# thomeou/SALSA

Hardware: AMD Instinct MI355X
Metric: SALSA feat-extract audio-s/s (higher is better)
Workload: dtype f64 (STFT, noise-floor tracker, eigen-solve cold list) + packed f32 (covariance and eigen-solve of the certified frames); 1 GPU; Full SALSA FOA (eigenvector path): batch 32x60-s 4-ch 24 kHz clips per GPU, feature-extract only, n_fft 512 hop 300 fmax_doa 9000 cond 5 tracking on; clips_per_gpu=32, feature=salsa, format=foa, clip_groups=default

## Files before the change

include/salsa_hip.h:

```cpp
#ifndef SALSA_HIP_H
#define SALSA_HIP_H

#include <stddef.h>
#include <stdint.h>

#ifdef __cplusplus
extern "C" {
#endif

#define SALSA_ABI_VERSION 2

enum { SALSA_FORMAT_FOA = 0, SALSA_FORMAT_MIC = 1 };
enum { SALSA_FEATURE_SALSA = 0, SALSA_FEATURE_LITE = 1, SALSA_FEATURE_IPD = 2 };
enum { SALSA_LAYOUT_PLANAR = 0, SALSA_LAYOUT_INTERLEAVED = 1 };

enum { SALSA_FLAG_FLEX = 1, SALSA_FLAG_NO_CLIP_FREQS = 2, SALSA_FLAG_CLIP_SPATIAL_ALIAS = 4,
       SALSA_FLAG_FORCE_F64 = 8 };

enum {
    SALSA_OK = 0,
    SALSA_PARTIAL = 1,
    SALSA_EINVAL = -1,
    SALSA_ENFFT = -2,
    SALSA_EFORMAT = -3,
// ... 41 lines not shown

int salsa_logspec_batch(salsa_plan *plan, const float *d_audio, int batch, int n_channels, int64_t n_samples,
                        float *d_out, void *hip_stream);

size_t salsa_eigvec_workspace_bytes(const salsa_plan *plan, int batch, int n_bins, int64_t n_frames);
int salsa_eigvec_batch(salsa_plan *plan, const float *d_X, int batch, int n_bins, int64_t n_frames, int lower_bin,
                       double *d_out, unsigned char *d_gate, void *d_workspace, size_t workspace_bytes,
                       void *hip_stream);

int salsa_eigvec_feature_batch(salsa_plan *plan, const float *d_X, int batch, int n_bins, int64_t n_frames, int lower_bin,
                               float *d_feat, void *d_workspace, size_t workspace_bytes, void *hip_stream);

int salsa_plan_set_fused(salsa_plan *plan, int mode);

int salsa_plan_set_stats(salsa_plan *plan, unsigned long long *d_counters);

int salsa_scaler_accumulate(const float *d_feat, int batch, int n_channels, int64_t n_frames, int n_freq,
                            int n_scaler_channels, double *d_sums, void *hip_stream);
int salsa_normalize_batch(float *d_feat, int batch, int n_channels, int64_t n_frames, int n_freq, int n_scaler_channels,
                          const float *d_mean, const float *d_std, void *hip_stream);

int salsa_plan_set_scaler(salsa_plan *plan, const float *d_mean, const float *d_std);

int salsa_to_freq_major(const float *d_feat, int64_t n_rows, int64_t n_frames, int n_freq, double *d_out, void *hip_stream);

#define SALSA_AUGMENT_NPAR 40
int salsa_augment_batch(const float *d_in, int64_t in_batch_stride, int64_t in_channel_stride, float *d_out, int batch,
                        int64_t n_frames, int n_freq, int audio_format, int n_zero_channels, const int *d_params,
                        const float *d_uval, const float *d_minmax, void *hip_stream);
int salsa_augment_gcc_batch(const float *d_in, int64_t in_batch_stride, int64_t in_channel_stride, float *d_out, int batch,
// ... 104 lines not shown
```

salsa_amd/csrc/build_guard.h:

```cpp
#ifndef SALSA_BUILD_GUARD_H
#define SALSA_BUILD_GUARD_H

#if !defined(SALSA_PROBE_BUILD)
#ifdef BN_PROBE_NO_Y
#error "BN_PROBE_NO_Y is a timing-probe switch: build with -DSALSA_PROBE_BUILD (its results are not the product's)"
#endif
#ifdef CONV_FETCH_COLMAJOR
#error "CONV_FETCH_COLMAJOR is a timing-probe switch: build with -DSALSA_PROBE_BUILD (its results are not the product's)"
#endif
#ifdef CONV_NO_BARRIER
#error "CONV_NO_BARRIER is a timing-probe switch: build with -DSALSA_PROBE_BUILD (its results are not the product's)"
#endif
#ifdef CONV_NO_EPI
#error "CONV_NO_EPI is a timing-probe switch: build with -DSALSA_PROBE_BUILD (its results are not the product's)"
#endif
#ifdef CONV_NO_FETCH
#error "CONV_NO_FETCH is a timing-probe switch: build with -DSALSA_PROBE_BUILD (its results are not the product's)"
#endif
#ifdef CONV_NO_LDSREAD
#error "CONV_NO_LDSREAD is a timing-probe switch: build with -DSALSA_PROBE_BUILD (its results are not the product's)"
#endif
#ifdef CONV_NO_ROW_SHARE
#error "CONV_NO_ROW_SHARE is a timing-probe switch: build with -DSALSA_PROBE_BUILD (its results are not the product's)"
#endif
// ... 21 lines not shown
#ifdef FZ_PROBE_NOSOLVE
#error "FZ_PROBE_NOSOLVE is a timing-probe switch: build with -DSALSA_PROBE_BUILD (its results are not the product's)"
#endif
#ifdef GRU_PROBE_BWD_NO_LOAD
#error "GRU_PROBE_BWD_NO_LOAD is a timing-probe switch: build with -DSALSA_PROBE_BUILD (its results are not the product's)"
#endif
#ifdef GRU_PROBE_BWD_NO_MATVEC
#error "GRU_PROBE_BWD_NO_MATVEC is a timing-probe switch: build with -DSALSA_PROBE_BUILD (its results are not the product's)"
#endif
#ifdef GRU_PROBE_BWD_NO_STORE
#error "GRU_PROBE_BWD_NO_STORE is a timing-probe switch: build with -DSALSA_PROBE_BUILD (its results are not the product's)"
#endif
#ifdef K1_FRAME_MAJOR
#error "K1_FRAME_MAJOR is a timing-probe switch: build with -DSALSA_PROBE_BUILD (its results are not the product's)"
#endif
#ifdef STEM_NO_STORE
#error "STEM_NO_STORE is a timing-probe switch: build with -DSALSA_PROBE_BUILD (its results are not the product's)"
#endif
#ifdef TR_PROBE_NO_CONSUME
#error "TR_PROBE_NO_CONSUME is a timing-probe switch: build with -DSALSA_PROBE_BUILD (its results are not the product's)"
#endif
#ifdef TR_PROBE_NO_PRODUCE
#error "TR_PROBE_NO_PRODUCE is a timing-probe switch: build with -DSALSA_PROBE_BUILD (its results are not the product's)"
#endif
#ifdef WIDE_W_ZERO
#error "WIDE_W_ZERO is a timing-probe switch: build with -DSALSA_PROBE_BUILD (its results are not the product's)"
#endif
#ifdef WIDE_X_ZERO
#error "WIDE_X_ZERO is a timing-probe switch: build with -DSALSA_PROBE_BUILD (its results are not the product's)"
#endif
// ... 203 lines not shown
#endif
#ifdef K1_NF_LITE
#define SALSA_BG_K1_NF_LITE " K1_NF_LITE=" SALSA_BG_STR(K1_NF_LITE)
#else
#define SALSA_BG_K1_NF_LITE ""
#endif
#ifdef K1_SPILL_NT
#define SALSA_BG_K1_SPILL_NT " K1_SPILL_NT=" SALSA_BG_STR(K1_SPILL_NT)
#else
#define SALSA_BG_K1_SPILL_NT ""
#endif
#ifdef K1_STD
#define SALSA_BG_K1_STD " K1_STD=" SALSA_BG_STR(K1_STD)
#else
#define SALSA_BG_K1_STD ""
#endif
#ifdef K3_FT_N
#define SALSA_BG_K3_FT_N " K3_FT_N=" SALSA_BG_STR(K3_FT_N)
#else
#define SALSA_BG_K3_FT_N ""
#endif
#ifdef K3_GATHER_NT
#define SALSA_BG_K3_GATHER_NT " K3_GATHER_NT=" SALSA_BG_STR(K3_GATHER_NT)
#else
#define SALSA_BG_K3_GATHER_NT ""
#endif
#ifdef K3_GROUP
#define SALSA_BG_K3_GROUP " K3_GROUP=" SALSA_BG_STR(K3_GROUP)
#else
#define SALSA_BG_K3_GROUP ""
// ... 213 lines not shown
    SALSA_BG_CONV_SPREAD_FETCH \
    SALSA_BG_CONV_STATS_DOT2 \
    SALSA_BG_CONV_WIDE_STORE \
    SALSA_BG_CONV_WPS \
    SALSA_BG_GRU_FILL \
    SALSA_BG_K1_INTERLEAVE \
    SALSA_BG_K1_LITE_1024_WAVES \
    SALSA_BG_K1_LITE_PAIR_MAJOR \
    SALSA_BG_K1_LITE_STD \
    SALSA_BG_K1_LITE_STD_WAVES \
    SALSA_BG_K1_LITE_WAVES \
    SALSA_BG_K1_NF_FULL \
    SALSA_BG_K1_NF_LITE \
    SALSA_BG_K1_SPILL_NT \
    SALSA_BG_K1_STD \
    SALSA_BG_K3_FT_N \
    SALSA_BG_K3_GATHER_NT \
    SALSA_BG_K3_GROUP \
    SALSA_BG_K3_NT_N \
    SALSA_BG_K3_OUT_NT \
    SALSA_BG_K3_PK_WAVES \
    SALSA_BG_K3_STAGE_LDS \
    SALSA_BG_K3_XCD_CHUNK \
    SALSA_BG_NN_NT_LD \
    SALSA_BG_NN_NT_ST \
    SALSA_BG_SALSA_COL0 \
    SALSA_BG_SALSA_COL0_MIN \
    SALSA_BG_SALSA_GATE_DOUBT \
    SALSA_BG_SALSA_PK \
    SALSA_BG_SALSA_PK_FOA_MIN \
// ... 29 lines not shown
```

salsa_amd/csrc/salsa_internal.h:

```cpp
#pragma once
#include <hip/hip_runtime.h>
#include <stdio.h>

#include "../../include/salsa_hip.h"
#include "salsa_math.h"
#include "salsa_workspace.h"

#define SALSA_LOCAL __attribute__((visibility("hidden")))

extern "C" SALSA_LOCAL void salsa_set_last_error_(const char *msg);

namespace salsa_impl {

static inline int fail(int code, const char *fmt, const char *a = "", long b = 0)
{
    char msg[512];
    snprintf(msg, sizeof(msg), fmt, a, b);
    salsa_set_last_error_(msg);
    return code;
}

static inline int hip_fail(const char *expr, hipError_t e)
{
    char msg[512];
// ... 26 lines not shown
    int format;
    int tracking;
    int n_hop;
    int pair_sel;
    int nch;
    double cond;
    double inv_cond;
    double delta;
    double snr_ratio;
    const float *sc_mean;
    const float *sc_std;
    unsigned long long *stats;
    int force_f64;
    unsigned *doubt32;
    unsigned *doubt_flag;
};

constexpr int FEATURE_LOGSPEC_ONLY = 3;

#ifndef K3_FT_N
#define K3_FT_N 8
#endif
constexpr int K3_FT = K3_FT_N;
#ifndef K3_NT_N
#define K3_NT_N 128
#endif
constexpr int K3_NT = K3_NT_N;
#ifndef SALSA_PK
#define SALSA_PK 1
#endif
#define SALSA_PK_COND_MIN 2.0

__device__ __forceinline__ int swz(int e) { return e ^ ((e >> 3) & 7); }

__device__ __forceinline__ void wave_lds_fence()
{
    __builtin_amdgcn_fence(__ATOMIC_RELEASE, "wavefront");
    __builtin_amdgcn_wave_barrier();
    __builtin_amdgcn_fence(__ATOMIC_ACQUIRE, "wavefront");
}

__device__ __forceinline__ float power32(const float2 x)
{
    const float t = x.x * x.x;
    return __builtin_fmaf(x.y, x.y, t);
}
// ... 11 lines not shown
}

constexpr int SALSA_MAX_GROUPS = 16;

struct salsa_plan {
    salsa_params p;
    int device;
    int lower, upper, cutoff, nd, F, ident;
    int spec_lo, spec_hi, flex;
    double delta, snr_ratio;
    double *d_window;
    double *d_window_doa;
    salsa::cplx<double> *d_tw;
    const float *sc_mean, *sc_std;
    unsigned long long *stats;
    int fused;
    int timing;
    int stop_after;
    int n_kernels;
    hipEvent_t ev0[SALSA_MAX_KERNELS], ev1[SALSA_MAX_KERNELS];
    const char *names[SALSA_MAX_KERNELS];
    int n_groups;
    int pipe_flags;
    hipStream_t streams[SALSA_MAX_GROUPS + 1];
    hipEvent_t ev_fork, ev_stft[SALSA_MAX_GROUPS], ev_stft2[SALSA_MAX_GROUPS], ev_join[SALSA_MAX_GROUPS + 1];
    hipStream_t cap_stream;
    hipGraphExec_t gexec;
    struct GraphKey {
        const float *audio;
        float *out;
        void *ws;
        const float *sc_mean, *sc_std;
        int batch, n_groups, flags;
        int64_t n_samples;
        bool operator==(const GraphKey &o) const
        {
            return audio == o.audio && out == o.out && ws == o.ws && sc_mean == o.sc_mean && sc_std == o.sc_std && batch == o.batch &&
                   n_groups == o.n_groups && flags == o.flags && n_samples == o.n_samples;
        }
    } gkey;
};

namespace salsa_impl {

static inline void bind_workspace(const WorkspaceLayout &L, void *base, int g0, bool with_doubt, float4 *&Xs, unsigned *&valid, KParams &kp)
{
    unsigned char *w = (unsigned char *)base;
    Xs = (float4 *)(w + L.spill_at(g0));
    valid = (unsigned *)(w + L.gate_at(g0));
    kp.doubt32 = with_doubt ? (unsigned *)(w + L.doubt_at(g0)) : nullptr;
    kp.doubt_flag = with_doubt ? (unsigned *)(w + L.flag_at(g0)) : nullptr;
}

// ... 35 lines not shown
```

salsa_amd/csrc/salsa_kernels.hip:

```cpp
#include "build_guard.h"
#include "salsa_internal.h"
#include <type_traits>

using salsa::cplx;
using namespace salsa_impl;

namespace {

template <int N> struct fft_cfg {
    static constexpr int NSUB = (N == 1024) ? 2 : 1;
    static constexpr int NS = N / NSUB;
    static constexpr int R = (NS == 512) ? 8 : 4;
    static constexpr int NP = (NS == 512) ? 2 : 3;
};

template <typename V> __device__ __forceinline__ V ld_off_c(const V *base, unsigned byte_off, int const_bytes) { return *(const V *)((const char *)base + byte_off + const_bytes); }
#ifndef K1_SPILL_NT
#define K1_SPILL_NT 1
#endif
typedef float salsa_f4v __attribute__((ext_vector_type(4)));
#ifndef TR_NT_LD
#define TR_NT_LD 0
#endif
#ifndef K3_GATHER_NT
// ... 644 lines not shown
#endif
constexpr int K3_OW = K3_NT + 8;
#ifndef K3_XCD_CHUNK
#define K3_XCD_CHUNK 16
#endif

#ifndef K3_STAGE_LDS
#define K3_STAGE_LDS 0
#endif
#ifndef K3_OUT_NT
#define K3_OUT_NT 1
#endif
#ifndef K3_PK_WAVES
#define K3_PK_WAVES 4
#endif
template <bool FEAT, int NHOP, bool FAST = false, bool PK = false>
__global__ __launch_bounds__(K3_NT, PK ? K3_PK_WAVES : 1) void cov_eig_kernel(const KParams kp, const float4 *__restrict__ Xs,
                                                      const unsigned *__restrict__ valid32,
                                                      float *__restrict__ out_feat, double *__restrict__ out_eig,
                                                      unsigned char *__restrict__ gate)
{
    constexpr int G = NHOP >= 0 ? K3_GROUP : 1;
    constexpr bool PAIRED = G > 1;
    static_assert(K3_FT % G == 0 && G <= 4 && K3_FT / G <= 16, "work-list entry layout");
    __shared__ unsigned short list[K3_FT * K3_NT];
    __shared__ unsigned short slow[FAST ? K3_FT * K3_NT : 1];
    __shared__ int count, nslow;
    __shared__ __attribute__((aligned(16))) unsigned rowoff[NHOP >= 0 ? K3_FT + 2 * NHOP + 2 : 2];
    __shared__ __attribute__((aligned(16))) float otile[FEAT ? 3 * K3_FT * K3_OW : 4];
#if K3_STAGE_LDS
// ... 98 lines not shown
        const int first = bin0 + K3_OW, tail = kp.F - first;
        for (int i = tid; i < nft * tail; i += K3_NT) {
            const int ft = i / tail, f = first + (i - ft * tail);
#pragma unroll
            for (int c = 0; c < 3; c++) st_off(of, 4u * (unsigned)((c * Tn + t0 + ft) * kp.F + f), 0.f);
        }
    }
    __syncthreads();
    const int n = count;
    const int stride = 2 * kp.nd;
    const int nhop = NHOP >= 0 ? NHOP : kp.n_hop;
    const float4 *xclip = Xs + (long)b * Tn * stride;
    const bool ungated = !kp.tracking && !kp.flex;
    auto solve_emit = [&](const salsa::herm4<double> &R, int t, int bin, auto path) {
        constexpr int PATH = decltype(path)::value;
        const bool foa = kp.format == SALSA_FORMAT_FOA;
        const salsa::eig_result<double> er = salsa::herm4_gate_eigvec<PATH>(R, kp.cond, kp.inv_cond, ungated, !foa);
        if (PATH == 1 && er.fallback) {
            slow[atomicAdd(&nslow, 1)] = (unsigned short)(((t - t0) << 8) | (bin - bin0));
            return;
        }
        if (er.doubt && kp.doubt32 && !ungated) {
            atomicOr(&kp.doubt32[((long)b * ((kp.nd + TR_BINS - 1) / TR_BINS) + (bin >> 5)) * Tn + t], 1u << (bin & 31));
            atomicOr(kp.doubt_flag, 1u);
        }
        double e[3] = {0.0, 0.0, 0.0};
        unsigned char g = er.rank1 ? 2 : 1;
        if (er.rank1 || ungated) {
            const int k = bin + kp.lower;
            const double den = kp.flex ? (double)((float)(k == 0 ? 1 : k) * (float)kp.delta) : kp.delta * (double)k;
            if (PATH != 2 && er.col0) {
                if (foa) salsa::normalise_foa_col0(er.u, e);
                else salsa::normalise_mic_col0(er.u, den, e);
            } else if (PATH != 1) {
                if (foa) salsa::normalise_foa(er.u, e, ungated);
                else salsa::normalise_mic(er.u, den, e);
            }
            g = 2;
        } else if (FEAT && kp.flex && !kp.tracking) {
            e[0] = __builtin_nan("");
        }
        emit(t, bin, e, g);
    };
    using hot_path = std::integral_constant<int, FAST ? 1 : 2>;
    using cold_path = std::integral_constant<int, 2>;
    if constexpr (PK) {
        static_assert(!PK || (G == 2 && FEAT && FAST && NHOP >= 0), "the packed solve takes the two frames of a pair");
        constexpr int NW = 2 * NHOP + 2;
        const unsigned half = 16u * (unsigned)kp.nd;
#if K3_STAGE_LDS
        if (n > 0) {
            for (int i = tid; i < (K3_FT + 6) * 2 * K3_NT; i += K3_NT) {
                const int fr = i / (2 * K3_NT), rem = i - fr * 2 * K3_NT, pr = rem / K3_NT, bl = rem - pr * K3_NT;
                if (bl < nbc) stage[i] = ld_off(xclip, rowoff[fr] + 16u * (unsigned)(bin0 + bl) + (pr ? half : 0u));
            }
// ... 99 lines not shown
        } else {
            salsa::herm4<double> R = {};
            for (int k = -nhop; k <= nhop; k++) {
                int tt = t + k;
                while (tt < 0) tt += Tn;
                while (tt >= Tn) tt -= Tn;
                const float4 a = xb[tt * stride], c = xb[tt * stride + kp.nd];
                const cplx<double> x[4] = {{(double)a.x, (double)a.y}, {(double)a.z, (double)a.w},
                                           {(double)c.x, (double)c.y}, {(double)c.z, (double)c.w}};
                salsa::herm4_rank1_add(R, x);
            }
            solve_emit(R, t, bin, hot_path{});
        }
    }
    if (FAST) {
        __syncthreads();
        const int ns = nslow;
        if (kp.stats && tid == 0) {
            int live = 0;
            for (int s = 0; s < n; s++) live += __popc((list[s] >> 12) & 15);
            atomicAdd(&kp.stats[0], (unsigned long long)n);
            atomicAdd(&kp.stats[1], (unsigned long long)live);
            atomicAdd(&kp.stats[2], (unsigned long long)ns);
            atomicAdd(&kp.stats[3], 1ull);
        }
        for (int s = tid; s < ns; s += K3_NT) {
            const int i = slow[s];
            const int t = t0 + (i >> 8), bin = bin0 + (i & 255);
            const float4 *xb = xclip + bin;
            salsa::herm4<double> R = {};
            for (int k = -nhop; k <= nhop; k++) {
                int tt = t + k;
                while (tt < 0) tt += Tn;
                while (tt >= Tn) tt -= Tn;
                const float4 a = xb[tt * stride], c = xb[tt * stride + kp.nd];
                const cplx<double> x[4] = {{(double)a.x, (double)a.y}, {(double)a.z, (double)a.w},
                                           {(double)c.x, (double)c.y}, {(double)c.z, (double)c.w}};
                salsa::herm4_rank1_add(R, x);
            }
            solve_emit(R, t, bin, cold_path{});
        }
    }
    if (FEAT) {
        __syncthreads();
        const bool vec = !(kp.F & 3) && !(seg & 3) && !(bin0 & 3);
        if (vec) {
            const int q = seg >> 2;
            for (int i = tid; i < 3 * nft * q; i += K3_NT) {
                const int row = i / q, col = i - row * q, c = row / nft, ft = row - c * nft;
                float4 *dst = (float4 *)(of + ((long)(c * Tn + t0 + ft) * kp.F + bin0 + 4 * col));
                const float4 val = *(const float4 *)(otile + (c * K3_FT + ft) * K3_OW + 4 * col);
                if (K3_OUT_NT) st_off_nt(dst, 0u, val);
                else *dst = val;
            }
        } else {
            for (int i = tid; i < 3 * nft * seg; i += K3_NT) {
                const int row = i / seg, col = i - row * seg, c = row / nft, ft = row - c * nft;
                of[(long)(c * Tn + t0 + ft) * kp.F + bin0 + col] = otile[(c * K3_FT + ft) * K3_OW + col];
            }
        }
    }
}

template <bool FEAT>
__global__ __launch_bounds__(256) void gate_doubt_kernel(const KParams kp, const float4 *__restrict__ Xs, float *__restrict__ out_feat,
                                                         double *__restrict__ out_eig, unsigned char *__restrict__ gate)
{
    if (*(const volatile unsigned *)kp.doubt_flag == 0u) return;
    const int Tn = kp.T, n32 = (kp.nd + TR_BINS - 1) / TR_BINS, stride = 2 * kp.nd;
    const long nwords = (long)kp.B * n32 * Tn;
    const bool foa = kp.format == SALSA_FORMAT_FOA;
    for (long wi = (long)blockIdx.x * blockDim.x + threadIdx.x; wi < nwords; wi += (long)gridDim.x * blockDim.x) {
        unsigned word = kp.doubt32[wi];
        if (!word) continue;
        const int t = (int)(wi % Tn), g32 = (int)((wi / Tn) % n32), b = (int)(wi / ((long)Tn * n32));
        while (word) {
            const int j = __ffs((int)word) - 1;
            word &= word - 1u;
            const int bin = 32 * g32 + j;
            const float4 *xb = Xs + (long)b * Tn * stride + bin;
            salsa::herm4<double> R = {};
            for (int k = -kp.n_hop; k <= kp.n_hop; k++) {
                int tt = t + k;
                while (tt < 0) tt += Tn;
                while (tt >= Tn) tt -= Tn;
                const float4 a = xb[tt * stride], c = xb[tt * stride + kp.nd];
                const cplx<double> x[4] = {{(double)a.x, (double)a.y}, {(double)a.z, (double)a.w},
                                           {(double)c.x, (double)c.y}, {(double)c.z, (double)c.w}};
                salsa::herm4_rank1_add(R, x);
            }
            const bool rank1 = salsa::herm4_rank1_by_jacobi(R, kp.cond);
            double e[3] = {0.0, 0.0, 0.0};
            if (rank1) {
                const salsa::eig_result<double> er = salsa::herm4_gate_eigvec<2>(R, kp.cond, kp.inv_cond, true, !foa);
                const int k = bin + kp.lower;
                const double den = kp.flex ? (double)((float)(k == 0 ? 1 : k) * (float)kp.delta) : kp.delta * (double)k;
                if (foa) salsa::normalise_foa(er.u, e, false);
                else salsa::normalise_mic(er.u, den, e);
            } else if (FEAT && kp.flex && !kp.tracking) {
                e[0] = __builtin_nan("");
            }
            if (FEAT) {
#pragma unroll
                for (int i = 0; i < 3; i++) out_feat[(((long)b * kp.OC + 4 + i) * Tn + t) * kp.F + bin] = (float)e[i];
            } else {
#pragma unroll
                for (int i = 0; i < 3; i++) out_eig[(((long)b * 3 + i) * kp.nd + bin) * Tn + t] = e[i];
                if (gate) gate[((long)b * kp.nd + bin) * Tn + t] = rank1 ? 2 : 1;
            }
        }
    }
}

__global__ __launch_bounds__(256) void flex_allpass_kernel(const KParams kp, float *__restrict__ out)
{
    const int bin = blockIdx.x * 256 + threadIdx.x;
    if (bin >= kp.nd) return;
    float *of = out + ((long)blockIdx.y * kp.OC + kp.nch) * kp.T * kp.F + bin;
    bool dead = false;
    for (int t = 0; t < kp.T; t++) {
        const float v = of[t * kp.F];
        dead = dead || (v != v);
        if (dead) {
            for (int c = 0; c < kp.nch - 1; c++) of[(c * kp.T + t) * kp.F] = 0.f;
        }
    }
}

}

namespace salsa_impl {

void launch_tracker(const KParams &kp, hipStream_t s, const float4 *Xs, unsigned *valid32)
{
    hipLaunchKernelGGL(tracker_kernel, dim3(tracker_grid(kp)), dim3(64 * TR_WAVES), 0, s, kp, Xs, valid32);
}

template <bool FEAT>
static void launch_gate_doubt(const KParams &kp, hipStream_t s, const float4 *Xs, float *out_feat, double *out_eig, unsigned char *gate)
{
    if (!kp.doubt32) return;
    const long nwords = (long)kp.B * ((kp.nd + TR_BINS - 1) / TR_BINS) * kp.T;
    const unsigned blocks = (unsigned)(nwords < 256L * 64 ? (nwords + 255) / 256 : 64);
    hipLaunchKernelGGL(gate_doubt_kernel<FEAT>, dim3(blocks ? blocks : 1u), dim3(256), 0, s, kp, Xs, out_feat, out_eig, gate);
}

template <bool FEAT>
void launch_cov_eig(const KParams &kp, dim3 grid, hipStream_t s, const float4 *Xs, const unsigned *valid,
                    float *out_feat, double *out_eig, unsigned char *gate)
{
    const bool gated = kp.tracking || kp.flex;
    if (kp.doubt32 && !kp.tracking) (void)hipMemsetAsync(kp.doubt_flag, 0, sizeof(unsigned), s);
    if (FEAT && SALSA_PK && K3_GROUP == 2 && kp.n_hop == 3 && gated && SALSA_COL0 && !kp.flex && kp.cond >= SALSA_PK_COND_MIN && kp.cond < 1e6 && !kp.force_f64)
        hipLaunchKernelGGL((cov_eig_kernel<FEAT, 3, true, FEAT && K3_GROUP == 2>), grid, dim3(K3_NT), 0, s, kp, Xs, valid, out_feat, out_eig, gate);
    else if (kp.n_hop == 3 && gated && SALSA_COL0)
        hipLaunchKernelGGL((cov_eig_kernel<FEAT, 3, true>), grid, dim3(K3_NT), 0, s, kp, Xs, valid, out_feat, out_eig, gate);
    else if (kp.n_hop == 3)
        hipLaunchKernelGGL((cov_eig_kernel<FEAT, 3>), grid, dim3(K3_NT), 0, s, kp, Xs, valid, out_feat, out_eig, gate);
    else
        hipLaunchKernelGGL((cov_eig_kernel<FEAT, -1>), grid, dim3(K3_NT), 0, s, kp, Xs, valid, out_feat, out_eig, gate);
    launch_gate_doubt<FEAT>(kp, s, Xs, out_feat, out_eig, gate);
}

template void launch_cov_eig<true>(const KParams &, dim3, hipStream_t, const float4 *, const unsigned *, float *, double *, unsigned char *);
template void launch_cov_eig<false>(const KParams &, dim3, hipStream_t, const float4 *, const unsigned *, float *, double *, unsigned char *);

void launch_flex_allpass(const KParams &kp, hipStream_t s, float *out)
{
    hipLaunchKernelGGL(flex_allpass_kernel, dim3((unsigned)((kp.nd + 255) / 256), (unsigned)kp.B), dim3(256), 0, s, kp, out);
}

int launch_stft(salsa_plan *pl, const KParams &kp, const double *win, const float *d_audio, float *d_out, float4 *Xs, hipStream_t s)
{
    const bool lite = kp.feature == SALSA_FEATURE_LITE || kp.feature == SALSA_FEATURE_IPD;
    const bool single = !lite && kp.pair_sel >= 0;
    constexpr int NF_FULL = k1_cfg<false>::NF, NF_LITE = k1_cfg<true>::NF, NF_PAIR = 2 * k1_cfg<false>::NF;
// ... 67 lines not shown
```

salsa_amd/csrc/salsa_plan.hip:

```cpp
#include "build_guard.h"
#include "salsa_internal.h"
#include <string.h>
#include <memory>
#include <vector>

using salsa::cplx;
using namespace salsa_impl;

namespace {

thread_local char g_err[512] = "";
constexpr double PI = 3.14159265358979323846;

}

namespace salsa_impl {

KParams make_kparams(const salsa_plan *pl, int batch, int64_t n_samples)
{
    KParams kp;
    memset(&kp, 0, sizeof(kp));
    kp.B = batch;
    kp.N = (int)n_samples;
    kp.T = (int)(1 + n_samples / pl->p.hop_len);
// ... 12 lines not shown
    kp.compress = pl->flex ? 0 : pl->p.is_compress_high_freq;
    kp.layout = pl->p.audio_layout;
    kp.feature = pl->p.feature_type;
    kp.format = pl->p.audio_format;
    kp.tracking = pl->p.is_tracking;
    kp.n_hop = pl->p.n_hopframes;
    kp.pair_sel = -1;
    kp.nch = 4;
    kp.cond = pl->p.cond_num;
    kp.inv_cond = pl->p.cond_num > 0 ? 1.0 / pl->p.cond_num : 0.0;
    kp.delta = pl->delta;
    kp.sc_mean = pl->sc_mean;
    kp.sc_std = pl->sc_std;
    kp.stats = pl->stats;
    kp.force_f64 = (pl->p.flags & SALSA_FLAG_FORCE_F64) != 0;
    return kp;
}

}

namespace {

static int mark_begin(salsa_plan *pl, hipStream_t s, const char *name)
{
    if (!pl->timing || pl->n_kernels >= SALSA_MAX_KERNELS) return -1;
    const int i = pl->n_kernels++;
    pl->names[i] = name;
    if (!pl->ev0[i]) (void)hipEventCreate(&pl->ev0[i]);
    if (!pl->ev1[i]) (void)hipEventCreate(&pl->ev1[i]);
    (void)hipEventRecord(pl->ev0[i], s);
// ... 90 lines not shown
        HIP_TRY(hipStreamWaitEvent(pl->streams[1 + g], pl->ev_fork, 0));
        const int g0 = (int)((long)batch * g / G), g1 = (int)((long)batch * (g + 1) / G);
        const int rc = issue_group(c, g0, g1, pl->streams[0], pl->streams[1 + g], pl->ev_stft[g], pl->ev_stft2[g], split);
        if (rc) return rc;
        HIP_TRY(hipEventRecord(pl->ev_join[1 + g], pl->streams[1 + g]));
        HIP_TRY(hipStreamWaitEvent(origin, pl->ev_join[1 + g], 0));
    }
    HIP_TRY(hipEventRecord(pl->ev_join[0], pl->streams[0]));
    HIP_TRY(hipStreamWaitEvent(origin, pl->ev_join[0], 0));
    return SALSA_OK;
}

static int replay_graph(const ExtractCall &c, int G, hipStream_t s)
{
    salsa_plan *pl = c.pl;
    const salsa_plan::GraphKey key = {c.audio, c.out, c.ws, pl->sc_mean, pl->sc_std, c.kp.B, G, pl->pipe_flags, (int64_t)c.kp.N};
    if (!(pl->gexec && pl->gkey == key)) {
        if (pl->gexec) {
            (void)hipGraphExecDestroy(pl->gexec);
            pl->gexec = nullptr;
        }
        hipGraph_t graph = nullptr;
        HIP_TRY(hipStreamBeginCapture(pl->cap_stream, hipStreamCaptureModeThreadLocal));
        const int rc = issue_forked(c, G, pl->cap_stream);
        const hipError_t e = hipStreamEndCapture(pl->cap_stream, &graph);
        if (rc) {
            if (graph) (void)hipGraphDestroy(graph);
            return rc;
        }
        HIP_TRY(e);
        const hipError_t ei = hipGraphInstantiate(&pl->gexec, graph, nullptr, nullptr, 0);
// ... 167 lines not shown
        return fail(SALSA_EFORMAT, "Unknown audio format%s");
    if (p.feature_type < SALSA_FEATURE_SALSA || p.feature_type > SALSA_FEATURE_IPD)
        return fail(SALSA_EINVAL, "Invalid feature type%s");
    if (p.feature_type != SALSA_FEATURE_SALSA && p.audio_format != SALSA_FORMAT_MIC)
        return fail(SALSA_EFORMAT, "SALSA-Lite and SALSA-IPD are only for MIC format!%s");
    if (p.n_hopframes < 0 || p.n_hopframes > 16) return fail(SALSA_EINVAL, "n_hopframes out of range%s");
    std::unique_ptr<salsa_plan, int (*)(salsa_plan *)> pl(new salsa_plan(), salsa_plan_destroy);
    memset(pl.get(), 0, sizeof(salsa_plan));
    pl->p = p;
    pl->flex = (p.flags & SALSA_FLAG_FLEX) != 0;
    pl->snr_ratio = p.floor_mask_ratio > 0 ? p.floor_mask_ratio : 1.5;
    if (const int rc = plan_bands(pl.get())) return rc;
    pl->delta = 2.0 * PI * p.fs / (p.n_fft * 343.0);
    if (hipGetDevice(&pl->device) != hipSuccess) return fail(SALSA_EHIP, "hipGetDevice failed (no HIP device?)%s");
    if (const int rc = plan_upload_tables(pl.get())) return rc;
    pl->n_groups = 1;
    *out_plan = pl.release();
    return SALSA_OK;
}

int salsa_plan_destroy(salsa_plan *pl)
{
    if (!pl) return SALSA_OK;
    if (pl->d_window) (void)hipFree(pl->d_window);
    if (pl->d_tw) (void)hipFree(pl->d_tw);
    for (int i = 0; i < SALSA_MAX_KERNELS; i++) {
        if (pl->ev0[i]) (void)hipEventDestroy(pl->ev0[i]);
        if (pl->ev1[i]) (void)hipEventDestroy(pl->ev1[i]);
    }
    for (int i = 0; i <= SALSA_MAX_GROUPS; i++) {
// ... 107 lines not shown

int salsa_plan_set_fused(salsa_plan *pl, int mode)
{
    if (!pl || mode < 0 || mode > 2) return fail(SALSA_EINVAL, "salsa_plan_set_fused: bad argument%s");
    pl->fused = mode;
    return SALSA_OK;
}

int salsa_plan_set_stats(salsa_plan *pl, unsigned long long *d_counters)
{
    if (!pl) return fail(SALSA_EINVAL, "salsa_plan_set_stats: NULL plan%s");
    pl->stats = d_counters;
    return SALSA_OK;
}

int salsa_plan_set_timing(salsa_plan *pl, int enable)
{
    if (!pl) return fail(SALSA_EINVAL, "salsa_plan_set_timing: NULL plan%s");
    pl->timing = enable > 0 ? enable : 0;
    pl->stop_after = enable < 0 ? (enable >= -2 ? -enable : 0) : 0;
    pl->n_kernels = 0;
    return SALSA_OK;
}

int salsa_plan_read_timing(salsa_plan *pl, float *ms, const char **names, int *n_out)
{
    if (!pl || !ms || !n_out) return fail(SALSA_EINVAL, "salsa_plan_read_timing: NULL argument%s");
    *n_out = 0;
    if (!pl->timing || pl->n_kernels == 0) return SALSA_OK;
    for (int i = 0; i < pl->n_kernels; i++) {
// ... 55 lines not shown
```

salsa_amd/extractor.py:

```python
import contextlib
import ctypes as C

import numpy as np
import torch

from . import _lib


def _raise(rc):
    msg = _lib.last_error()
    if rc == _lib.E_NFFT:
        raise AssertionError(msg)
    if rc == _lib.E_FORMAT:
        if 'only for MIC' in msg:
            raise AssertionError(msg)
        raise ValueError(msg)
    if rc == _lib.E_BINS:
        raise AssertionError(msg)
    if rc == _lib.E_INVAL:
        raise ValueError(msg)
    raise RuntimeError('libsalsa_hip: %s (code %d)' % (msg, rc))


def bin_limits(fs, n_fft, fmin_doa, fmax_doa):
# ... 34 lines not shown
            audio_layout=_lib.LAYOUT[audio_layout], flags=int(flags), floor_mask_ratio=float(floor_mask_ratio),
            fmax_spec=int(fmax_spec), reserved=0)
        self.audio_layout = audio_layout
        self.feature_type = feature_type
        self._plan = C.c_void_p()
        with torch.cuda.device(self.device):
            rc = self.L.salsa_plan_create(C.byref(self.params), C.byref(self._plan))
        if rc:
            self._plan = None
            _raise(rc)
        self._ws = None
        self._prefix_mode = False
        self._scaler = None
        self._pipe = None
        self._stats = None
        self._fused = 0

    def copy_plan_state_to(self, other: 'SalsaExtractor'):
        if self._scaler is not None:
            other.set_scaler(*self._scaler)
        else:
            other.set_scaler(None)
        if self._pipe is not None:
            other.set_pipeline(*self._pipe)
        if self._fused != other._fused:
            other.set_fused(self._fused)

    def kwargs(self):
        p = self.params
        inv = lambda d, v: [k for k, x in d.items() if x == v][0]
        return dict(fs=p.fs, n_fft=p.n_fft, hop_len=p.hop_len, win_len=p.win_len, fmin_doa=p.fmin_doa, fmax_doa=p.fmax_doa,
                    cond_num=p.cond_num, n_hopframes=p.n_hopframes, is_tracking=bool(p.is_tracking),
                    is_compress_high_freq=bool(p.is_compress_high_freq), audio_format=inv(_lib.FORMAT, p.audio_format),
                    feature_type=self.feature_type, audio_layout=self.audio_layout, device=self.device, flags=p.flags,
                    floor_mask_ratio=p.floor_mask_ratio, fmax_spec=p.fmax_spec)

    def __del__(self):
        if getattr(self, '_plan', None):
            self.L.salsa_plan_destroy(self._plan)
            self._plan = None

# ... 100 lines not shown
                                                   self._stream())
        if rc:
            _raise(rc)
        return feat[:, 4:]

    def set_fused(self, mode: int):
        rc = self.L.salsa_plan_set_fused(self._plan, int(mode))
        if rc:
            _raise(rc)
        self._fused = int(mode)

    def set_stats(self, on: bool = True):
        if not on:
            torch.cuda.synchronize(self.device)
        self._stats = torch.zeros(4, dtype=torch.int64, device=self.device) if on else None
        rc = self.L.salsa_plan_set_stats(self._plan, C.c_void_p(self._stats.data_ptr()) if on else None)
        if rc:
            _raise(rc)

    def read_stats(self):
        if self._stats is None:
            raise RuntimeError('read_stats(): no counters attached -- call set_stats(True) first')
        v = self._stats.cpu().tolist()
        self._stats.zero_()
        return dict(items=v[0], gated_frames=v[1], cold_frames=v[2], tiles=v[3])

    def set_timing(self, enable):
        if int(enable) < 0:
            raise ValueError('set_timing takes 0, 1 or a repeat count; the prefix-issue measurement mode is issue_prefix()')
        self.L.salsa_plan_set_timing(self._plan, int(enable))

    @contextlib.contextmanager
    def issue_prefix(self, kernels: int):
        assert kernels in (1, 2)
        self.L.salsa_plan_set_timing(self._plan, -kernels)
        self._prefix_mode = True
        try:
            yield self
        finally:
            self._prefix_mode = False
# ... 169 lines not shown
```

Measured before the change: 2.080 million audio-seconds/s.

## Add optional deferral of small cold lists to a compacted gate-doubt pass

```diff
diff --git a/include/salsa_hip.h b/include/salsa_hip.h
--- a/include/salsa_hip.h
+++ b/include/salsa_hip.h
@@ -79,6 +79,10 @@
 int salsa_plan_set_fused(salsa_plan *plan, int mode);
 
 int salsa_plan_set_stats(salsa_plan *plan, unsigned long long *d_counters);
+
+int salsa_plan_set_cold_defer(salsa_plan *plan, int defer_max);
+
+int salsa_plan_set_cold_defer_stats(salsa_plan *plan, unsigned long long *d_counters);
 
 int salsa_scaler_accumulate(const float *d_feat, int batch, int n_channels, int64_t n_frames, int n_freq,
                             int n_scaler_channels, double *d_sums, void *hip_stream);
diff --git a/salsa_amd/csrc/build_guard.h b/salsa_amd/csrc/build_guard.h
--- a/salsa_amd/csrc/build_guard.h
+++ b/salsa_amd/csrc/build_guard.h
@@ -59,6 +59,9 @@
 #ifdef K1_FRAME_MAJOR
 #error "K1_FRAME_MAJOR is a timing-probe switch: build with -DSALSA_PROBE_BUILD (its results are not the product's)"
 #endif
+#ifdef K3_PROBE_NO_COLD
+#error "K3_PROBE_NO_COLD is a timing-probe switch: build with -DSALSA_PROBE_BUILD (its results are not the product's)"
+#endif
 #ifdef STEM_NO_STORE
 #error "STEM_NO_STORE is a timing-probe switch: build with -DSALSA_PROBE_BUILD (its results are not the product's)"
 #endif
@@ -292,6 +295,11 @@
 #define SALSA_BG_K1_STD " K1_STD=" SALSA_BG_STR(K1_STD)
 #else
 #define SALSA_BG_K1_STD ""
+#endif
+#ifdef K3_COLD_DEFER
+#define SALSA_BG_K3_COLD_DEFER " K3_COLD_DEFER=" SALSA_BG_STR(K3_COLD_DEFER)
+#else
+#define SALSA_BG_K3_COLD_DEFER ""
 #endif
 #ifdef K3_FT_N
 #define SALSA_BG_K3_FT_N " K3_FT_N=" SALSA_BG_STR(K3_FT_N)
@@ -535,6 +543,7 @@
     SALSA_BG_K1_NF_LITE \
     SALSA_BG_K1_SPILL_NT \
     SALSA_BG_K1_STD \
+    SALSA_BG_K3_COLD_DEFER \
     SALSA_BG_K3_FT_N \
     SALSA_BG_K3_GATHER_NT \
     SALSA_BG_K3_GROUP \
diff --git a/salsa_amd/csrc/salsa_internal.h b/salsa_amd/csrc/salsa_internal.h
--- a/salsa_amd/csrc/salsa_internal.h
+++ b/salsa_amd/csrc/salsa_internal.h
@@ -64,6 +64,9 @@
     int force_f64;
     unsigned *doubt32;
     unsigned *doubt_flag;
+    int cold_defer;
+    int n_cu;
+    unsigned long long *defer_stats;
 };
 
 constexpr int FEATURE_LOGSPEC_ONLY = 3;
@@ -80,6 +83,10 @@
 #define SALSA_PK 1
 #endif
 #define SALSA_PK_COND_MIN 2.0
+#ifndef K3_COLD_DEFER
+#define K3_COLD_DEFER 0
+#endif
+constexpr int COLD_DEFER_DEFAULT = K3_COLD_DEFER;
 
 __device__ __forceinline__ int swz(int e) { return e ^ ((e >> 3) & 7); }
 
@@ -121,6 +128,9 @@
     salsa::cplx<double> *d_tw;
     const float *sc_mean, *sc_std;
     unsigned long long *stats;
+    unsigned long long *defer_stats;
+    int cold_defer;
+    int n_cu;
     int fused;
     int timing;
     int stop_after;
@@ -140,10 +150,11 @@
         const float *sc_mean, *sc_std;
         int batch, n_groups, flags;
         int64_t n_samples;
+        int cold_defer;
         bool operator==(const GraphKey &o) const
         {
             return audio == o.audio && out == o.out && ws == o.ws && sc_mean == o.sc_mean && sc_std == o.sc_std && batch == o.batch &&
-                   n_groups == o.n_groups && flags == o.flags && n_samples == o.n_samples;
+                   n_groups == o.n_groups && flags == o.flags && n_samples == o.n_samples && cold_defer == o.cold_defer;
         }
     } gkey;
 };
diff --git a/salsa_amd/csrc/salsa_kernels.hip b/salsa_amd/csrc/salsa_kernels.hip
--- a/salsa_amd/csrc/salsa_kernels.hip
+++ b/salsa_amd/csrc/salsa_kernels.hip
@@ -682,6 +682,46 @@
 #ifndef K3_PK_WAVES
 #define K3_PK_WAVES 4
 #endif
+template <int NW, int UNR, typename Off, typename Row>
+__device__ __forceinline__ salsa::herm4<double> cold_cov(const float4 *xclip, Row row, Off boff, Off half)
+{
+    salsa::herm4<double> R = {};
+#pragma unroll UNR
+    for (int k = 0; k < NW; k++) {
+        const Off r = row(k) + boff;
+        const float4 a = *(const float4 *)((const char *)xclip + r), c = *(const float4 *)((const char *)xclip + (r + half));
+        const cplx<double> x[4] = {{(double)a.x, (double)a.y}, {(double)a.z, (double)a.w},
+                                   {(double)c.x, (double)c.y}, {(double)c.z, (double)c.w}};
+        salsa::herm4_rank1_add(R, x);
+    }
+    return R;
+}
+template <int PATH, bool FEAT>
+__device__ __forceinline__ salsa::eig_result<double> solve_bin(const KParams &kp, const salsa::herm4<double> &R, int bin, bool ungated,
+                                                                double *e, unsigned char &g)
+{
+    const bool foa = kp.format == SALSA_FORMAT_FOA;
+    const salsa::eig_result<double> er = salsa::herm4_gate_eigvec<PATH>(R, kp.cond, kp.inv_cond, ungated, !foa);
+    e[0] = e[1] = e[2] = 0.0;
+    g = er.rank1 ? 2 : 1;
+    if (PATH == 1 && er.fallback) return er;
+    if (er.rank1 || ungated) {
+        const int k = bin + kp.lower;
+        const double den = kp.flex ? (double)((float)(k == 0 ? 1 : k) * (float)kp.delta) : kp.delta * (double)k;
+        if (PATH != 2 && er.col0) {
+            if (foa) salsa::normalise_foa_col0(er.u, e);
+            else salsa::normalise_mic_col0(er.u, den, e);
+        } else if (PATH != 1) {
+            if (foa) salsa::normalise_foa(er.u, e, ungated);
+            else salsa::normalise_mic(er.u, den, e);
+        }
+        g = 2;
+    } else if (FEAT && kp.flex && !kp.tracking) {
+        e[0] = __builtin_nan("");
+    }
+    return er;
+}
+
 template <bool FEAT, int NHOP, bool FAST = false, bool PK = false>
 __global__ __launch_bounds__(K3_NT, PK ? K3_PK_WAVES : 1) void cov_eig_kernel(const KParams kp, const float4 *__restrict__ Xs,
                                                       const unsigned *__restrict__ valid32,
@@ -810,8 +850,9 @@
     const bool ungated = !kp.tracking && !kp.flex;
     auto solve_emit = [&](const salsa::herm4<double> &R, int t, int bin, auto path) {
         constexpr int PATH = decltype(path)::value;
-        const bool foa = kp.format == SALSA_FORMAT_FOA;
-        const salsa::eig_result<double> er = salsa::herm4_gate_eigvec<PATH>(R, kp.cond, kp.inv_cond, ungated, !foa);
+        double e[3];
+        unsigned char g;
+        const salsa::eig_result<double> er = solve_bin<PATH, FEAT>(kp, R, bin, ungated, e, g);
         if (PATH == 1 && er.fallback) {
             slow[atomicAdd(&nslow, 1)] = (unsigned short)(((t - t0) << 8) | (bin - bin0));
             return;
@@ -819,22 +860,6 @@
         if (er.doubt && kp.doubt32 && !ungated) {
             atomicOr(&kp.doubt32[((long)b * ((kp.nd + TR_BINS - 1) / TR_BINS) + (bin >> 5)) * Tn + t], 1u << (bin & 31));
             atomicOr(kp.doubt_flag, 1u);
-        }
-        double e[3] = {0.0, 0.0, 0.0};
-        unsigned char g = er.rank1 ? 2 : 1;
-        if (er.rank1 || ungated) {
-            const int k = bin + kp.lower;
-            const double den = kp.flex ? (double)((float)(k == 0 ? 1 : k) * (float)kp.delta) : kp.delta * (double)k;
-            if (PATH != 2 && er.col0) {
-                if (foa) salsa::normalise_foa_col0(er.u, e);
-                else salsa::normalise_mic_col0(er.u, den, e);
-            } else if (PATH != 1) {
-                if (foa) salsa::normalise_foa(er.u, e, ungated);
-                else salsa::normalise_mic(er.u, den, e);
-            }
-            g = 2;
-        } else if (FEAT && kp.flex && !kp.tracking) {
-            e[0] = __builtin_nan("");
         }
         emit(t, bin, e, g);
     };
@@ -964,8 +989,13 @@
         }
     }
     if (FAST) {
+        static_assert(!FAST || NHOP >= 0, "the cold loop reads its window through rowoff");
         __syncthreads();
+#ifdef K3_PROBE_NO_COLD
+        const int ns = 0;
+#else
         const int ns = nslow;
+#endif
         if (kp.stats && tid == 0) {
             int live = 0;
             for (int s = 0; s < n; s++) live += __popc((list[s] >> 12) & 15);
@@ -974,21 +1004,29 @@
             atomicAdd(&kp.stats[2], (unsigned long long)ns);
             atomicAdd(&kp.stats[3], 1ull);
         }
-        for (int s = tid; s < ns; s += K3_NT) {
-            const int i = slow[s];
-            const int t = t0 + (i >> 8), bin = bin0 + (i & 255);
-            const float4 *xb = xclip + bin;
-            salsa::herm4<double> R = {};
-            for (int k = -nhop; k <= nhop; k++) {
-                int tt = t + k;
-                while (tt < 0) tt += Tn;
-                while (tt >= Tn) tt -= Tn;
-                const float4 a = xb[tt * stride], c = xb[tt * stride + kp.nd];
-                const cplx<double> x[4] = {{(double)a.x, (double)a.y}, {(double)a.z, (double)a.w},
-                                           {(double)c.x, (double)c.y}, {(double)c.z, (double)c.w}};
-                salsa::herm4_rank1_add(R, x);
-            }
-            solve_emit(R, t, bin, cold_path{});
+        if (PK && kp.doubt32 && ns > 0 && ns <= kp.cold_defer) {
+            const int n32 = (kp.nd + TR_BINS - 1) / TR_BINS;
+            for (int s = tid; s < ns; s += K3_NT) {
+                const int i = slow[s];
+                const int t = t0 + (i >> 8), bin = bin0 + (i & 255);
+                atomicOr(&kp.doubt32[((long)b * n32 + (bin >> 5)) * Tn + t], 1u << (bin & 31));
+            }
+            if (tid == 0) {
+                atomicOr(kp.doubt_flag, 1u);
+                if (kp.defer_stats) {
+                    atomicAdd(&kp.defer_stats[0], (unsigned long long)ns);
+                    atomicAdd(&kp.defer_stats[1], 1ull);
+                }
+            }
+        } else {
+            for (int s = tid; s < ns; s += K3_NT) {
+                const int i = slow[s];
+                const int ft = i >> 8, bin = bin0 + (i & 255);
+                const unsigned *ro = rowoff + ft;
+                const salsa::herm4<double> R =
+                    cold_cov<2 * (NHOP >= 0 ? NHOP : 0) + 1, 4>(xclip, [&](int k) { return ro[k]; }, 16u * (unsigned)bin, 16u * (unsigned)kp.nd);
+                solve_emit(R, t0 + ft, bin, cold_path{});
+            }
         }
     }
     if (FEAT) {
@@ -1012,43 +1050,99 @@
     }
 }
 
-template <bool FEAT>
-__global__ __launch_bounds__(256) void gate_doubt_kernel(const KParams kp, const float4 *__restrict__ Xs, float *__restrict__ out_feat,
-                                                         double *__restrict__ out_eig, unsigned char *__restrict__ gate)
+constexpr int GD_NT = 256;
+constexpr int GD_QCAP = GD_NT * 32 + GD_NT;
+template <bool FEAT, int NHOP>
+__global__ __launch_bounds__(GD_NT) void gate_doubt_kernel(const KParams kp, const float4 *__restrict__ Xs, float *__restrict__ out_feat,
+                                                           double *__restrict__ out_eig, unsigned char *__restrict__ gate, const int deferring)
 {
     if (*(const volatile unsigned *)kp.doubt_flag == 0u) return;
+    __shared__ unsigned queue[GD_QCAP];
+    __shared__ int qn;
+    const int tid = threadIdx.x, lane = tid & 63;
     const int Tn = kp.T, n32 = (kp.nd + TR_BINS - 1) / TR_BINS, stride = 2 * kp.nd;
     const long nwords = (long)kp.B * n32 * Tn;
+    const long nstep = (nwords + GD_NT - 1) / GD_NT;
     const bool foa = kp.format == SALSA_FORMAT_FOA;
-    for (long wi = (long)blockIdx.x * blockDim.x + threadIdx.x; wi < nwords; wi += (long)gridDim.x * blockDim.x) {
-        unsigned word = kp.doubt32[wi];
-        if (!word) continue;
-        const int t = (int)(wi % Tn), g32 = (int)((wi / Tn) % n32), b = (int)(wi / ((long)Tn * n32));
-        while (word) {
-            const int j = __ffs((int)word) - 1;
-            word &= word - 1u;
-            const int bin = 32 * g32 + j;
-            const float4 *xb = Xs + (long)b * Tn * stride + bin;
-            salsa::herm4<double> R = {};
-            for (int k = -kp.n_hop; k <= kp.n_hop; k++) {
-                int tt = t + k;
-                while (tt < 0) tt += Tn;
-                while (tt >= Tn) tt -= Tn;
-                const float4 a = xb[tt * stride], c = xb[tt * stride + kp.nd];
-                const cplx<double> x[4] = {{(double)a.x, (double)a.y}, {(double)a.z, (double)a.w},
-                                           {(double)c.x, (double)c.y}, {(double)c.z, (double)c.w}};
-                salsa::herm4_rank1_add(R, x);
-            }
-            const bool rank1 = salsa::herm4_rank1_by_jacobi(R, kp.cond);
+    const bool ungated = !kp.tracking && !kp.flex;
+    if (tid == 0) qn = 0;
+    __syncthreads();
+    auto load_step = [&](long c) { return c < nstep && c * GD_NT + tid < nwords ? kp.doubt32[c * GD_NT + tid] : 0u; };
+    unsigned ahead = load_step(blockIdx.x);
+    unsigned k = 0;
+    for (long c = blockIdx.x; c < nstep; c += gridDim.x, k++) {
+        const unsigned word = ahead;
+        ahead = load_step(c + gridDim.x);
+        const unsigned long long nz = __ballot(word != 0u);
+        if (nz) {
+            int total = 0;
+            for (unsigned long long m = nz; m; m &= m - 1)
+                total += __popc((unsigned)__builtin_amdgcn_readlane((int)word, __builtin_amdgcn_readfirstlane(__builtin_ctzll(m))));
+            int base = 0;
+            if (lane == 0) base = atomicAdd(&qn, total);
+            base = __builtin_amdgcn_readfirstlane(base);
+            const unsigned first = k * GD_NT + (unsigned)(tid - lane);
+            for (unsigned long long m = nz; m; m &= m - 1) {
+                const int l = __builtin_amdgcn_readfirstlane(__builtin_ctzll(m));
+                const unsigned w = (unsigned)__builtin_amdgcn_readlane((int)word, l);
+                if (lane < 32 && ((w >> lane) & 1u)) queue[base + __popc(w & ((1u << lane) - 1u))] = ((first + (unsigned)l) << 5) | (unsigned)lane;
+                base += __popc(w);
+            }
+        }
+        __syncthreads();
+        const int n = qn;
+        __syncthreads();
+        if (n < GD_NT && c + gridDim.x < nstep) continue;
+        if (tid == 0) qn = 0;
+        for (int s = tid; s < n; s += GD_NT) {
+            const unsigned q = queue[s];
+            const long w = ((long)blockIdx.x + (long)(q >> 13) * gridDim.x) * GD_NT + (long)((q >> 5) & (GD_NT - 1));
+            const int t = (int)(w % Tn), g32 = (int)((w / Tn) % n32), b = (int)(w / ((long)Tn * n32));
+            const int bin = 32 * g32 + (int)(q & 31u);
+            const float4 *xclip = Xs + (long)b * Tn * stride;
+            salsa::herm4<double> R;
+            if constexpr (NHOP >= 0) {
+                size_t rows[2 * NHOP + 1];
+#pragma unroll
+                for (int k = 0; k <= 2 * NHOP; k++) {
+                    int tt = t - NHOP + k;
+                    while (tt < 0) tt += Tn;
+                    while (tt >= Tn) tt -= Tn;
+                    rows[k] = (size_t)tt * (size_t)stride * sizeof(float4);
+                }
+                R = cold_cov<2 * NHOP + 1, 2 * NHOP + 1>(xclip, [&](int k) { return rows[k]; }, sizeof(float4) * (size_t)bin,
+                                                            sizeof(float4) * (size_t)kp.nd);
+            } else {
+                R = {};
+                const float4 *xb = xclip + bin;
+                for (int k = -kp.n_hop; k <= kp.n_hop; k++) {
+                    int tt = t + k;
+                    while (tt < 0) tt += Tn;
+                    while (tt >= Tn) tt -= Tn;
+                    const float4 a = xb[(long)tt * stride], c = xb[(long)tt * stride + kp.nd];
+                    const cplx<double> x[4] = {{(double)a.x, (double)a.y}, {(double)a.z, (double)a.w},
+                                               {(double)c.x, (double)c.y}, {(double)c.z, (double)c.w}};
+                    salsa::herm4_rank1_add(R, x);
+                }
+            }
             double e[3] = {0.0, 0.0, 0.0};
-            if (rank1) {
-                const salsa::eig_result<double> er = salsa::herm4_gate_eigvec<2>(R, kp.cond, kp.inv_cond, true, !foa);
-                const int k = bin + kp.lower;
-                const double den = kp.flex ? (double)((float)(k == 0 ? 1 : k) * (float)kp.delta) : kp.delta * (double)k;
-                if (foa) salsa::normalise_foa(er.u, e, false);
-                else salsa::normalise_mic(er.u, den, e);
-            } else if (FEAT && kp.flex && !kp.tracking) {
-                e[0] = __builtin_nan("");
+            unsigned char g = 1;
+            bool doubt = true;
+            if (deferring) doubt = solve_bin<2, FEAT>(kp, R, bin, ungated, e, g).doubt && !ungated;
+            if (doubt) {
+                if (kp.defer_stats) atomicAdd(&kp.defer_stats[2], 1ull);
+                const bool rank1 = salsa::herm4_rank1_by_jacobi(R, kp.cond);
+                e[0] = e[1] = e[2] = 0.0;
+                g = rank1 ? 2 : 1;
+                if (rank1) {
+                    const salsa::eig_result<double> er = salsa::herm4_gate_eigvec<2>(R, kp.cond, kp.inv_cond, true, !foa);
+                    const int k = bin + kp.lower;
+                    const double den = kp.flex ? (double)((float)(k == 0 ? 1 : k) * (float)kp.delta) : kp.delta * (double)k;
+                    if (foa) salsa::normalise_foa(er.u, e, false);
+                    else salsa::normalise_mic(er.u, den, e);
+                } else if (FEAT && kp.flex && !kp.tracking) {
+                    e[0] = __builtin_nan("");
+                }
             }
             if (FEAT) {
 #pragma unroll
@@ -1056,9 +1150,10 @@
             } else {
 #pragma unroll
                 for (int i = 0; i < 3; i++) out_eig[(((long)b * 3 + i) * kp.nd + bin) * Tn + t] = e[i];
-                if (gate) gate[((long)b * kp.nd + bin) * Tn + t] = rank1 ? 2 : 1;
-            }
-        }
+                if (gate) gate[((long)b * kp.nd + bin) * Tn + t] = g;
+            }
+        }
+        __syncthreads();
     }
 }
 
@@ -1087,12 +1182,16 @@
 }
 
 template <bool FEAT>
-static void launch_gate_doubt(const KParams &kp, hipStream_t s, const float4 *Xs, float *out_feat, double *out_eig, unsigned char *gate)
+static void launch_gate_doubt(const KParams &kp, hipStream_t s, const float4 *Xs, float *out_feat, double *out_eig, unsigned char *gate, bool deferring)
 {
     if (!kp.doubt32) return;
     const long nwords = (long)kp.B * ((kp.nd + TR_BINS - 1) / TR_BINS) * kp.T;
-    const unsigned blocks = (unsigned)(nwords < 256L * 64 ? (nwords + 255) / 256 : 64);
-    hipLaunchKernelGGL(gate_doubt_kernel<FEAT>, dim3(blocks ? blocks : 1u), dim3(256), 0, s, kp, Xs, out_feat, out_eig, gate);
+    const long steps = (nwords + GD_NT - 1) / GD_NT, cap = deferring ? 4L * (kp.n_cu > 0 ? kp.n_cu : 64) : 64L;
+    const dim3 grid((unsigned)(steps < 1 ? 1 : steps < cap ? steps : cap));
+    if (kp.n_hop == 3)
+        hipLaunchKernelGGL((gate_doubt_kernel<FEAT, 3>), grid, dim3(GD_NT), 0, s, kp, Xs, out_feat, out_eig, gate, (int)deferring);
+    else
+        hipLaunchKernelGGL((gate_doubt_kernel<FEAT, -1>), grid, dim3(GD_NT), 0, s, kp, Xs, out_feat, out_eig, gate, (int)deferring);
 }
 
 template <bool FEAT>
@@ -1101,7 +1200,9 @@
 {
     const bool gated = kp.tracking || kp.flex;
     if (kp.doubt32 && !kp.tracking) (void)hipMemsetAsync(kp.doubt_flag, 0, sizeof(unsigned), s);
-    if (FEAT && SALSA_PK && K3_GROUP == 2 && kp.n_hop == 3 && gated && SALSA_COL0 && !kp.flex && kp.cond >= SALSA_PK_COND_MIN && kp.cond < 1e6 && !kp.force_f64)
+    const bool packed = FEAT && SALSA_PK && K3_GROUP == 2 && kp.n_hop == 3 && gated && SALSA_COL0 && !kp.flex && kp.cond >= SALSA_PK_COND_MIN &&
+                        kp.cond < 1e6 && !kp.force_f64;
+    if (packed)
         hipLaunchKernelGGL((cov_eig_kernel<FEAT, 3, true, FEAT && K3_GROUP == 2>), grid, dim3(K3_NT), 0, s, kp, Xs, valid, out_feat, out_eig, gate);
     else if (kp.n_hop == 3 && gated && SALSA_COL0)
         hipLaunchKernelGGL((cov_eig_kernel<FEAT, 3, true>), grid, dim3(K3_NT), 0, s, kp, Xs, valid, out_feat, out_eig, gate);
@@ -1109,7 +1210,7 @@
         hipLaunchKernelGGL((cov_eig_kernel<FEAT, 3>), grid, dim3(K3_NT), 0, s, kp, Xs, valid, out_feat, out_eig, gate);
     else
         hipLaunchKernelGGL((cov_eig_kernel<FEAT, -1>), grid, dim3(K3_NT), 0, s, kp, Xs, valid, out_feat, out_eig, gate);
-    launch_gate_doubt<FEAT>(kp, s, Xs, out_feat, out_eig, gate);
+    launch_gate_doubt<FEAT>(kp, s, Xs, out_feat, out_eig, gate, packed && kp.cold_defer > 0);
 }
 
 template void launch_cov_eig<true>(const KParams &, dim3, hipStream_t, const float4 *, const unsigned *, float *, double *, unsigned char *);
diff --git a/salsa_amd/csrc/salsa_plan.hip b/salsa_amd/csrc/salsa_plan.hip
--- a/salsa_amd/csrc/salsa_plan.hip
+++ b/salsa_amd/csrc/salsa_plan.hip
@@ -50,6 +50,9 @@
     kp.sc_std = pl->sc_std;
     kp.stats = pl->stats;
     kp.force_f64 = (pl->p.flags & SALSA_FLAG_FORCE_F64) != 0;
+    kp.cold_defer = pl->cold_defer;
+    kp.n_cu = pl->n_cu;
+    kp.defer_stats = pl->defer_stats;
     return kp;
 }
 
@@ -170,7 +173,8 @@
 static int replay_graph(const ExtractCall &c, int G, hipStream_t s)
 {
     salsa_plan *pl = c.pl;
-    const salsa_plan::GraphKey key = {c.audio, c.out, c.ws, pl->sc_mean, pl->sc_std, c.kp.B, G, pl->pipe_flags, (int64_t)c.kp.N};
+    const salsa_plan::GraphKey key = {c.audio, c.out, c.ws, pl->sc_mean, pl->sc_std, c.kp.B, G, pl->pipe_flags, (int64_t)c.kp.N,
+                                      pl->cold_defer};
     if (!(pl->gexec && pl->gkey == key)) {
         if (pl->gexec) {
             (void)hipGraphExecDestroy(pl->gexec);
@@ -368,6 +372,9 @@
     pl->delta = 2.0 * PI * p.fs / (p.n_fft * 343.0);
     if (hipGetDevice(&pl->device) != hipSuccess) return fail(SALSA_EHIP, "hipGetDevice failed (no HIP device?)%s");
     if (const int rc = plan_upload_tables(pl.get())) return rc;
+    if (hipDeviceGetAttribute(&pl->n_cu, hipDeviceAttributeMultiprocessorCount, pl->device) != hipSuccess || pl->n_cu <= 0)
+        return fail(SALSA_EHIP, "hipDeviceGetAttribute(multiprocessor count) failed%s");
+    pl->cold_defer = COLD_DEFER_DEFAULT;
     pl->n_groups = 1;
     *out_plan = pl.release();
     return SALSA_OK;
@@ -505,6 +512,20 @@
     return SALSA_OK;
 }
 
+int salsa_plan_set_cold_defer(salsa_plan *pl, int defer_max)
+{
+    if (!pl || defer_max < 0) return fail(SALSA_EINVAL, "salsa_plan_set_cold_defer: bad argument%s");
+    pl->cold_defer = defer_max;
+    return SALSA_OK;
+}
+
+int salsa_plan_set_cold_defer_stats(salsa_plan *pl, unsigned long long *d_counters)
+{
+    if (!pl) return fail(SALSA_EINVAL, "salsa_plan_set_cold_defer_stats: NULL plan%s");
+    pl->defer_stats = d_counters;
+    return SALSA_OK;
+}
+
 int salsa_plan_set_timing(salsa_plan *pl, int enable)
 {
     if (!pl) return fail(SALSA_EINVAL, "salsa_plan_set_timing: NULL plan%s");
diff --git a/salsa_amd/extractor.py b/salsa_amd/extractor.py
--- a/salsa_amd/extractor.py
+++ b/salsa_amd/extractor.py
@@ -72,6 +72,8 @@
         self._scaler = None
         self._pipe = None
         self._stats = None
+        self._defer_stats = None
+        self._cold_defer = None
         self._fused = 0
 
     def copy_plan_state_to(self, other: 'SalsaExtractor'):
@@ -83,6 +85,8 @@
             other.set_pipeline(*self._pipe)
         if self._fused != other._fused:
             other.set_fused(self._fused)
+        if self._cold_defer is not None:
+            other.set_cold_defer(self._cold_defer)
 
     def kwargs(self):
         p = self.params
@@ -213,7 +217,11 @@
         if not on:
             torch.cuda.synchronize(self.device)
         self._stats = torch.zeros(4, dtype=torch.int64, device=self.device) if on else None
+        self._defer_stats = torch.zeros(3, dtype=torch.int64, device=self.device) if on else None
         rc = self.L.salsa_plan_set_stats(self._plan, C.c_void_p(self._stats.data_ptr()) if on else None)
+        if rc:
+            _raise(rc)
+        rc = self.L.salsa_plan_set_cold_defer_stats(self._plan, C.c_void_p(self._defer_stats.data_ptr()) if on else None)
         if rc:
             _raise(rc)
 
@@ -223,6 +231,21 @@
         v = self._stats.cpu().tolist()
         self._stats.zero_()
         return dict(items=v[0], gated_frames=v[1], cold_frames=v[2], tiles=v[3])
+
+    COLD_DEFER_ALL = 2 ** 31 - 1
+
+    def set_cold_defer(self, defer_max):
+        rc = self.L.salsa_plan_set_cold_defer(self._plan, self.COLD_DEFER_ALL if defer_max == 'all' else int(defer_max))
+        if rc:
+            _raise(rc)
+        self._cold_defer = defer_max
+
+    def read_defer_stats(self):
+        if self._defer_stats is None:
+            raise RuntimeError('read_defer_stats(): no counters attached -- call set_stats(True) first')
+        v = self._defer_stats.cpu().tolist()
+        self._defer_stats.zero_()
+        return dict(deferred_frames=v[0], deferring_tiles=v[1], jacobi_bins=v[2])
 
     def set_timing(self, enable):
         if int(enable) < 0:
```

Result: no change. 2.087 million audio-seconds/s (median of 3 runs) (+0.3%).
